# lbcb-sci/raven

Hardware: NVIDIA H100
Metric: overlaps/s (higher is better)
Workload: dtype u64

## Files before the change

raven_b200/csrc/capi.cu:

```cuda
#include <algorithm>
#include <cstring>

#include "engine.cuh"

using namespace rvn;

struct rvn_ctx {
  Ctx c;
};

namespace {

template <typename F>
int Guard(rvn_ctx* ctx, F&& f, bool sketches_first = false) {
  if (!ctx) return RVN_ERR_INVALID;
  try {
    RVN_CUDA(cudaSetDevice(ctx->c.device));
    if (!sketches_first) WaitUpload(ctx->c);
    f(ctx->c);
    ctx->c.err.clear();
    return RVN_OK;
  } catch (const InvalidArgument& e) {
    ctx->c.err = e.what();
    return RVN_ERR_INVALID;
// ... 677 lines not shown
    if (!out) throw InvalidArgument("null stats");
    *out = c.stats;
    out->occurrence = c.occurrence;
    out->kernel_launches = c.launches;
  }, true);
}

RVN_API int rvn_set_option(rvn_ctx* ctx, const char* name, int64_t value) {
  return Guard(ctx, [&](Ctx& c) {
    if (name && std::strcmp(name, "keep_hits") == 0) {
      c.keep_hits = value != 0;
    } else if (name && std::strcmp(name, "async_upload") == 0) {
      c.async_upload = value != 0;
    } else if (name && std::strcmp(name, "self_join") == 0) {
      c.self_join = value != 0;
    } else if (name && std::strcmp(name, "tier_min_records") == 0) {
      c.tier_min_records = value < 0 ? 0 : static_cast<uint64_t>(value);
    } else if (name && std::strcmp(name, "reset_stats") == 0) {
      std::memset(&c.stats, 0, sizeof(c.stats));
      c.launches = 0;
      TimerReset(c);
    } else {
      throw InvalidArgument("unknown option");
    }
  }, true);
}

RVN_API int rvn_get_timings(rvn_ctx* ctx, const char* const** names,
                            const float** ms, uint32_t* n) {
  return Guard(ctx, [&](Ctx& c) {
// ... 203 lines not shown
```

raven_b200/csrc/engine.cuh:

```cuda
#pragma once

#include <string>
#include <vector>

#include "../../include/raven_b200.h"
#include "common.cuh"

namespace rvn {

struct Params {
  uint32_t k = 15, w = 5, bandwidth = 500, chain = 4, matches = 100;
  uint32_t gap = 10000;
};

constexpr uint32_t kSketchTile = 2048;
constexpr uint32_t kSketchThreads = 256;
constexpr uint32_t kMaxWindow = 256;

struct PhaseTimer {
  std::vector<const char*> names;
  std::vector<float> ms;
  std::vector<std::pair<cudaEvent_t, cudaEvent_t>> pending;
  std::vector<cudaEvent_t> pool;
};
// ... 40 lines not shown

  bool q_valid = false;
  uint32_t q_first = 0, q_last = 0;
  uint64_t q_n = 0;
  DevBuf<uint64_t> q_val, q_org, q_off;
  bool q_is32 = false;
  std::vector<uint64_t> h_q_off;
  bool qt_valid = false;
  uint32_t qt_first = 0, qt_last = 0;
  DevBuf<uint64_t> qt_val;
  DevBuf<uint32_t> qt_pos;
  int t_b_low = 0;
  uint64_t group_count_min = 0;
  bool i_from_sketch = false;
  int64_t self_join = 1;

  bool i_valid = false;
  uint32_t i_first = 0, i_last = 0;
  uint64_t i_n = 0, i_keys = 0;
  DevBuf<uint64_t> i_val, i_org, i_val_alt, i_org_alt;
  bool i_is32 = false;
  int i_shift = 0;
  uint64_t i_limit = ~0ULL;
  DevBuf<uint32_t> t_cnt;
  DevBuf<uint64_t> t_off, t_aval, t_aorg, t_b0, t_b1, t_b2, t_narrow;
  const uint32_t* t_sorted_b = nullptr;
  uint64_t t_nb = 0;
  uint64_t tier_min_records = 1ULL << 18;
  DevBuf<uint32_t> i_bucket;
  int i_bucket_bits = 0;
  DevBuf<uint64_t> i_gaps;
  DevBuf<uint64_t> i_hist;
  uint32_t occurrence = 0xFFFFFFFFu;
  bool i_sorted_ids = false;
  bool ids_ascending = true;
  DevBuf<uint8_t> sort_tmp;

  DevBuf<uint32_t> m_cnt, m_first;
  DevBuf<uint8_t> m_filt;
  DevBuf<uint64_t> m_hit_off;
  DevBuf<uint64_t> m_sq_key, m_sq_key2;
  DevBuf<uint32_t> m_sq_idx, m_sq_idx2;
// ... 91 lines not shown
void TimerBegin(Ctx& c, const char* name);
void TimerEnd(Ctx& c);
void TimerCollect(Ctx& c);
void TimerReset(Ctx& c);

void EnsureTiles(Ctx& c);
void EnsureSketch(Ctx& c, uint32_t first, uint32_t last);
void WaitUpload(Ctx& c);
void EnsureMicromizers(Ctx& c, uint32_t first, uint32_t last);
void EnsureThresholds(Ctx& c, uint32_t first, uint32_t last);

void BuildIndex(Ctx& c, uint32_t first, uint32_t last, bool minhash,
                uint64_t value_limit = ~0ULL);
uint64_t MaxMicromizerValue(Ctx& c, uint32_t first, uint32_t last);
void BuildIndexFrom(Ctx& c, ValView src_val, const uint64_t* src_org, uint64_t n,
                    uint64_t index_bases, uint64_t value_limit = ~0ULL);

int RadixSortPairs(Ctx& c, const uint32_t* src_keys, uint32_t* keys_a, uint32_t* keys_b,
                   const uint64_t* src_vals, uint64_t* vals_a, uint64_t* vals_b, uint64_t n,
                   int begin_bit, int end_bit, bool descending = false);
int RadixSortPairs(Ctx& c, const uint64_t* src_keys, uint64_t* keys_a, uint64_t* keys_b,
                   const uint64_t* src_vals, uint64_t* vals_a, uint64_t* vals_b, uint64_t n,
                   int begin_bit, int end_bit, bool descending = false);
int RadixSortPairs(Ctx& c, const uint32_t* src_keys, uint32_t* keys_a, uint32_t* keys_b,
                   const uint32_t* src_vals, uint32_t* vals_a, uint32_t* vals_b, uint64_t n,
                   int begin_bit, int end_bit, bool descending = false);
int RadixSortPairs(Ctx& c, const uint64_t* src_keys, uint64_t* keys_a, uint64_t* keys_b,
                   const uint32_t* src_vals, uint32_t* vals_a, uint32_t* vals_b, uint64_t n,
                   int begin_bit, int end_bit, bool descending = false);
int RadixSortKeys(Ctx& c, const uint32_t* src_keys, uint32_t* keys_a, uint32_t* keys_b,
                  uint64_t n, int begin_bit, int end_bit);
uint64_t* IndexHistogram(Ctx& c);
uint32_t ThresholdFromHistogram(Ctx& c, const uint64_t* h_hist, uint64_t n_keys,
                                double frequency, bool* needs_long_runs);
uint32_t FilterIndex(Ctx& c, double frequency);

void MapRange(Ctx& c, uint32_t first, uint32_t last, bool avoid_equal,
              bool avoid_symmetric, bool minhash, bool want_filtered,
              bool fetch = true);

uint64_t ChainGroupedHits(Ctx& c, const uint64_t* hg, const uint64_t* hp,
                          const uint64_t* read_hit_off,
                          const std::vector<uint64_t>& h_rho, const uint32_t* lhs_ids,
                          uint32_t nr, uint64_t n_hits, uint64_t n_q);

void GatherReset(Ctx& c);
// ... 52 lines not shown
```

raven_b200/csrc/index.cu:

```cuda
#include <algorithm>
#include <cmath>

#include "engine.cuh"

namespace rvn {

namespace {

constexpr int kThreads = 256;

constexpr uint32_t kHistBins = 1u << 16;
constexpr uint32_t kSmemBins = 1024;

constexpr uint32_t kShortGap = 1024;
constexpr uint32_t kMaxLongGaps = 1u << 20;

template <typename ValT, bool kFill>
__global__ void __launch_bounds__(kThreads)
IndexTableKernel(const ValT* __restrict__ val, uint64_t n, int shift,
                 uint32_t n_buckets, uint32_t* __restrict__ bucket,
                 unsigned long long* __restrict__ hist, uint64_t* __restrict__ gaps) {
  __shared__ uint32_t sh[kSmemBins];
  __shared__ uint32_t keys;
  __shared__ uint32_t warp_first[kThreads / 32];
// ... 313 lines not shown
    atomicAdd(&sh[1], h1);
    atomicAdd(&sh[2], h2);
    atomicAdd(&sh[3], h3);
    atomicAdd(&sh[4], h4);
    atomicAdd(&keys_total, nkeys);
  }
  __syncthreads();
  for (uint32_t i = threadIdx.x; i < kSmemBins; i += kThreads) {
    if (sh[i]) atomicAdd(&hist[i], static_cast<unsigned long long>(sh[i]));
  }
  if (threadIdx.x == 0 && keys_total) {
    atomicAdd(&hist[kHistBins], static_cast<unsigned long long>(keys_total));
  }
}

}

uint64_t MaxMicromizerValue(Ctx& c, uint32_t first, uint32_t last) {
  EnsureThresholds(c, first, last);
  if (last <= first) return 0;
  if (!c.s_is32) return ~0ULL;
  uint64_t* w = c.m_counter.reserve(8);
  RVN_CUDA(cudaMemsetAsync(w, 0, sizeof(uint64_t), c.stream));
  const uint64_t n = last - first;
  MaxU64Kernel<<<std::min<unsigned>(CeilDiv(n, 256), c.sms * 8), 256, 0, c.stream>>>(
      c.qt_val.get(), n, reinterpret_cast<unsigned long long*>(w));
  RVN_LAUNCH_CHECK();
  ++c.launches;
  return ReadU64(c, w);
}
// ... 3 lines not shown
  c.occurrence = 0xFFFFFFFFu;
  EnsureSketch(c, first, last);
  ValView src_val{c.s_val.get(), c.s_is32 ? 1 : 0};
  const uint64_t* src_org = c.s_org.get();
  uint64_t n = c.s_n;
  if (minhash) {
    EnsureMicromizers(c, first, last);
    src_val = ValView{c.q_val.get(), c.q_is32 ? 1 : 0};
    src_org = c.q_org.get();
    n = c.q_n;
  }
  uint64_t bases = 0;
  for (uint32_t r = first; r < last; ++r) bases += c.h_len[r];
  c.i_first = first;
  c.i_last = last;
  BuildIndexFrom(c, src_val, src_org, n, bases, minhash ? ~0ULL : value_limit);
  c.i_sorted_ids = c.ids_ascending;
  c.i_from_sketch = !minhash;
}

void BuildIndexFrom(Ctx& c, ValView src_val, const uint64_t* src_org, uint64_t n,
                    uint64_t index_bases, uint64_t value_limit) {
  c.i_valid = false;
  c.i_sorted_ids = false;
  c.i_from_sketch = false;
  c.occurrence = 0xFFFFFFFFu;
  ++c.i_gen;
  if (n >= 0xFFFFFFFFULL) {
    throw LimitError("index batch holds 2^32 or more minimizers");
  }
  c.i_n = n;
  c.i_keys = 0;
  if (!src_val.is32 && 2 * c.prm.k <= 30 && n > 0) {
    uint32_t* narrow = reinterpret_cast<uint32_t*>(c.t_narrow.reserve(n / 2 + 2));
    NarrowValuesKernel<<<CeilDiv(n, kThreads), kThreads, 0, c.stream>>>(
        static_cast<const uint64_t*>(src_val.p), n, narrow);
    RVN_LAUNCH_CHECK();
    ++c.launches;
    src_val = ValView{narrow, 1};
  }
  const bool is32 = src_val.is32 != 0;
  c.i_is32 = is32;

  const int key_bits = static_cast<int>(2 * c.prm.k);
  const uint64_t value_mask = key_bits >= 64 ? ~0ULL : ((1ULL << key_bits) - 1);
  const bool tiered = is32 && value_limit < value_mask && n >= c.tier_min_records;
  const uint32_t limit32 = static_cast<uint32_t>(value_limit);
  c.i_limit = tiered ? value_limit : ~0ULL;
  uint64_t n_a = n, n_b = 0;
  const uint32_t* sorted_b = nullptr;

  TimerBegin(c, "index_sort");
  if (tiered) {
    const uint32_t* src32 = static_cast<const uint32_t*>(src_val.p);
    const uint64_t tiles = (n + kTierTile - 1) / kTierTile;
    uint32_t* tcnt = c.t_cnt.reserve(tiles + 1);
    uint64_t* toff = c.t_off.reserve(tiles + 2);
    TierCountKernel<<<static_cast<unsigned>(tiles), kThreads, 0, c.stream>>>(src32, n, limit32,
                                                                          tcnt);
    ExclusiveScanU32(c, tcnt, toff, tiles);
    n_a = ReadU64(c, toff + tiles);
    n_b = n - n_a;
    uint32_t* a_val = reinterpret_cast<uint32_t*>(c.t_aval.reserve(n_a / 2 + 2));
    uint64_t* a_org = c.t_aorg.reserve(n_a + 1);
    uint32_t* b_src = reinterpret_cast<uint32_t*>(c.t_b0.reserve(n_b / 2 + 2));
// ... 5 lines not shown
    while (bits_a < key_bits && (value_limit >> bits_a) != 0) ++bits_a;
    c.i_val.reserve(n_a / 2 + 2);
    c.i_val_alt.reserve(n_a / 2 + 2);
    c.i_org.reserve(n_a + 1);
    c.i_org_alt.reserve(n_a + 1);
    if (n_a > 0) {
      const int where = RadixSortPairs(c, a_val, reinterpret_cast<uint32_t*>(c.i_val.get()),
                                       reinterpret_cast<uint32_t*>(c.i_val_alt.get()), a_org,
                                       c.i_org.get(), c.i_org_alt.get(), n_a, 0, bits_a);
      if (where == 1) {
        c.i_val.swap(c.i_val_alt);
        c.i_org.swap(c.i_org_alt);
      }
    }
    uint32_t* b1 = reinterpret_cast<uint32_t*>(c.t_b1.reserve(n_b / 2 + 2));
    uint32_t* b2 = reinterpret_cast<uint32_t*>(c.t_b2.reserve(n_b / 2 + 2));
    const uint64_t n_groups = ((value_mask - value_limit) >> kGroupLowBits) + 1;
    c.t_b_low = (key_bits > 2 * kGroupLowBits && n_b / n_groups >= c.group_count_min)
                    ? kGroupLowBits
                    : 0;
    if (n_b > 0) {
      const int where = RadixSortKeys(c, b_src, b1, b2, n_b, c.t_b_low, key_bits);
      sorted_b = where < 0 ? b_src : (where == 0 ? b1 : b2);
    }
    c.t_sorted_b = sorted_b;
    c.t_nb = n_b;
  } else {
    const uint64_t val_elems = is32 ? n / 2 + 2 : n + 1;
    c.i_val.reserve(val_elems);
    c.i_val_alt.reserve(val_elems);
    c.i_org.reserve(n + 1);
    c.i_org_alt.reserve(n + 1);
    if (n > 0) {
      int where;
      if (is32) {
        where = RadixSortPairs(c, static_cast<const uint32_t*>(src_val.p),
                               reinterpret_cast<uint32_t*>(c.i_val.get()),
                               reinterpret_cast<uint32_t*>(c.i_val_alt.get()), src_org,
                               c.i_org.get(), c.i_org_alt.get(), n, 0, key_bits);
      } else {
        where = RadixSortPairs(c, static_cast<const uint64_t*>(src_val.p), c.i_val.get(),
                               c.i_val_alt.get(), src_org, c.i_org.get(), c.i_org_alt.get(), n, 0,
                               key_bits);
      }
      if (where == 1) {
        c.i_val.swap(c.i_val_alt);
        c.i_org.swap(c.i_org_alt);
      }
    }
    c.t_sorted_b = nullptr;
    c.t_nb = 0;
  }
  c.i_n = n_a;
  TimerEnd(c);
  const uint64_t* kv = c.i_val.get();

  TimerBegin(c, "index_table");
  int top_bits = key_bits;
  if (tiered) {
    top_bits = 1;
    while (top_bits < key_bits && (value_limit >> top_bits) != 0) ++top_bits;
  }
  int bits = 8;
  while (bits < 28 && (1ULL << (bits + 1)) <= n_a) ++bits;
  bits = std::min<int>(bits, top_bits);
  c.i_bucket_bits = bits;
  const int shift = top_bits - bits;
  c.i_shift = shift;
  const uint32_t n_buckets =
      tiered ? static_cast<uint32_t>((value_limit >> shift) + 1) : (1u << bits);
  uint32_t* bucket = c.i_bucket.reserve(n_buckets + 2ULL);
  static_assert(sizeof(unsigned long long) == sizeof(uint64_t), "");
  uint64_t* hist = c.i_hist.reserve(kHistBins + 8);
  RVN_CUDA(cudaMemsetAsync(hist, 0, (kHistBins + 8) * sizeof(uint64_t), c.stream));
  uint64_t* gaps = c.i_gaps.reserve(3ULL * kMaxLongGaps);
  const unsigned grid = std::min<unsigned>(CeilDiv(n_a + 1, kThreads), c.sms * 8);
  if (is32) {
    IndexTableKernel<uint32_t, true><<<grid, kThreads, 0, c.stream>>>(
        reinterpret_cast<const uint32_t*>(kv), n_a, shift, n_buckets, bucket,
        reinterpret_cast<unsigned long long*>(hist), gaps);
    if (tiered && n_b > 0) {
      if (c.t_b_low) {
        GroupCountKernel<<<std::min<unsigned>(CeilDiv(n_b, kGroupChunk * (kThreads / 32)), c.sms * 6),
                           kThreads, 0, c.stream>>>(sorted_b, n_b,
                                                    reinterpret_cast<unsigned long long*>(hist));
      } else {
        IndexTableKernel<uint32_t, false>
            <<<std::min<unsigned>(CeilDiv(n_b + 1, kThreads), c.sms * 8), kThreads, 0, c.stream>>>(
                sorted_b, n_b, 0, 0, nullptr, reinterpret_cast<unsigned long long*>(hist), nullptr);
      }
      ++c.launches;
    }
  } else {
    IndexTableKernel<uint64_t, true><<<grid, kThreads, 0, c.stream>>>(
        kv, n_a, shift, n_buckets, bucket, reinterpret_cast<unsigned long long*>(hist), gaps);
  }
  RVN_LAUNCH_CHECK();
// ... 54 lines not shown
  bool long_runs = false;
  uint32_t occ = ThresholdFromHistogram(c, h.data(), c.i_keys, frequency, &long_runs);
  if (long_runs) {
    uint64_t cum = 0;
    for (uint32_t len = 0; len + 1 < kHistBins; ++len) cum += h[len];
    std::size_t rank = static_cast<std::size_t>((1 - frequency) * static_cast<double>(c.i_keys));
    if (rank >= c.i_keys) rank = c.i_keys - 1;
    const uint64_t n_long = h[kHistBins - 1];
    uint32_t* out = c.m_cnt.reserve(n_long + 1);
    uint64_t* counter = c.m_counter.reserve(8);
    RVN_CUDA(cudaMemsetAsync(counter, 0, sizeof(uint64_t), c.stream));
    if (c.i_is32) {
      CollectLongRuns<uint32_t><<<CeilDiv(c.i_n, kThreads), kThreads, 0, c.stream>>>(
          reinterpret_cast<const uint32_t*>(c.i_val.get()), c.i_n,
          reinterpret_cast<unsigned long long*>(counter), out);
      if (c.t_sorted_b && c.t_nb && c.t_b_low) {
        uint32_t* bufs[3] = {reinterpret_cast<uint32_t*>(c.t_b0.get()),
                             reinterpret_cast<uint32_t*>(c.t_b1.get()),
                             reinterpret_cast<uint32_t*>(c.t_b2.get())};
        uint32_t* free_buf[2];
        int nf = 0;
        for (uint32_t* p : bufs) {
          if (p != c.t_sorted_b && nf < 2) free_buf[nf++] = p;
        }
        const int where = RadixSortKeys(c, c.t_sorted_b, free_buf[0], free_buf[1], c.t_nb, 0,
                                        static_cast<int>(2 * c.prm.k));
        c.t_sorted_b = where < 0 ? c.t_sorted_b : (where == 0 ? free_buf[0] : free_buf[1]);
        c.t_b_low = 0;
      }
      if (c.t_sorted_b && c.t_nb) {
        CollectLongRuns<uint32_t><<<CeilDiv(c.t_nb, kThreads), kThreads, 0, c.stream>>>(
            c.t_sorted_b, c.t_nb, reinterpret_cast<unsigned long long*>(counter), out);
      }
    } else {
      CollectLongRuns<uint64_t><<<CeilDiv(c.i_n, kThreads), kThreads, 0, c.stream>>>(
          c.i_val.get(), c.i_n, reinterpret_cast<unsigned long long*>(counter), out);
    }
    RVN_LAUNCH_CHECK();
    ++c.launches;
    std::vector<uint32_t> lens(n_long);
    RVN_CUDA(cudaMemcpyAsync(lens.data(), out, n_long * sizeof(uint32_t),
                             cudaMemcpyDeviceToHost, c.stream));
    RVN_CUDA(cudaStreamSynchronize(c.stream));
// ... 10 lines not shown
```

raven_b200/csrc/radix.cu:

```cuda
#include <algorithm>

#include "engine.cuh"

namespace rvn {

namespace {

constexpr int kRadixMaxBits = 10;
constexpr int kBins = 1 << kRadixMaxBits;
constexpr int kThreads = 256;
constexpr int kWarps = kThreads / 32;
constexpr int kBinsPerThread = kBins / kThreads;
constexpr int kMaxPasses = 8;
template <typename KeyT>
struct Items {
  static constexpr int value = sizeof(KeyT) == 4 ? 32 : 16;
};

constexpr uint32_t kFlagAggregate = 1u << 30;
constexpr uint32_t kFlagPrefix = 2u << 30;
constexpr uint32_t kFlagMask = 3u << 30;
constexpr uint32_t kValueMask = ~kFlagMask;

struct PassPlan {
// ... 31 lines not shown
  for (int i = threadIdx.x; i < total; i += kThreads) {
    if (sh_hist[i]) atomicAdd(&hist[i], static_cast<unsigned long long>(sh_hist[i]));
  }
}

__global__ void __launch_bounds__(kBins)
RadixScanBinsKernel(const unsigned long long* __restrict__ hist, int n_passes,
                    uint32_t* __restrict__ bin_base) {
  __shared__ uint32_t sm[34];
  for (int p = 0; p < n_passes; ++p) {
    const uint32_t v = static_cast<uint32_t>(hist[p * kBins + threadIdx.x]);
    uint32_t total;
    const uint32_t ex = BlockExclusiveSum<uint32_t, kBins>(v, sm, &total);
    bin_base[p * kBins + threadIdx.x] = ex;
  }
}

template <typename KeyT, typename ValT, bool HAS_VAL>
struct __align__(16) PassSmem {
  static constexpr int kTile = kThreads * Items<KeyT>::value;
  uint16_t warp_hist[kWarps][kBins];
  uint32_t bin_off[kBins];
  uint32_t bin_dst[kBins];
  uint32_t scan[34];
  uint32_t tile;
  uint16_t slot_digit[HAS_VAL ? kTile : 2];
  union {
    KeyT keys[kTile];
    ValT vals[HAS_VAL ? kTile : 1];
  } stage;
// ... 85 lines not shown
      sm.warp_hist[w][b] = static_cast<uint16_t>(c);
      c += x;
    }
    cnt[j] = c;
    mine += c;
  }
  uint32_t total;
  uint32_t ex = BlockExclusiveSum<uint32_t, kThreads>(mine, sm.scan, &total);
#pragma unroll
  for (int j = 0; j < kBinsPerThread; ++j) {
    sm.bin_off[threadIdx.x * kBinsPerThread + j] = ex;
    ex += cnt[j];
  }

  {
    uint4* st4 = reinterpret_cast<uint4*>(status);
    const uint64_t my4 = static_cast<uint64_t>(tile) * (kBins / 4) + threadIdx.x;
    uint32_t excl[kBinsPerThread] = {0, 0, 0, 0};
    static_assert(kBinsPerThread == 4, "one uint4 of status words per thread");
    if (tile > 0) {
      uint4 agg;
      agg.x = kFlagAggregate | cnt[0];
      agg.y = kFlagAggregate | cnt[1];
      agg.z = kFlagAggregate | cnt[2];
      agg.w = kFlagAggregate | cnt[3];
      asm volatile("st.volatile.global.v4.u32 [%0], {%1, %2, %3, %4};" ::"l"(st4 + my4),
                   "r"(agg.x), "r"(agg.y), "r"(agg.z), "r"(agg.w)
                   : "memory");
      constexpr int kLook = 4;
      uint32_t open = 0xF;
      int64_t p = static_cast<int64_t>(tile) - 1;
      while (open) {
        uint4 v[kLook];
#pragma unroll
        for (int u = 0; u < kLook; ++u) {
          const int64_t q = p - u;
          if (q >= 0) {
            const uint4* src = st4 + static_cast<uint64_t>(q) * (kBins / 4) + threadIdx.x;
            asm volatile("ld.volatile.global.v4.u32 {%0, %1, %2, %3}, [%4];"
                         : "=r"(v[u].x), "=r"(v[u].y), "=r"(v[u].z), "=r"(v[u].w)
                         : "l"(src)
                         : "memory");
          } else {
            v[u] = make_uint4(kFlagPrefix, kFlagPrefix, kFlagPrefix, kFlagPrefix);
          }
        }
        int used = 0;
#pragma unroll
        for (int u = 0; u < kLook; ++u) {
          const uint32_t vv[4] = {v[u].x, v[u].y, v[u].z, v[u].w};
          const bool ready = (vv[0] & kFlagMask) && (vv[1] & kFlagMask) && (vv[2] & kFlagMask) &&
                             (vv[3] & kFlagMask);
          if (used == u && ready && open) {
#pragma unroll
            for (int j = 0; j < kBinsPerThread; ++j) {
              if (open & (1u << j)) {
                excl[j] += vv[j] & kValueMask;
                if ((vv[j] & kFlagMask) == kFlagPrefix) open &= ~(1u << j);
              }
            }
            used = u + 1;
          }
        }
        p -= used;
      }
    }
    uint4 pre;
    pre.x = kFlagPrefix | (excl[0] + cnt[0]);
    pre.y = kFlagPrefix | (excl[1] + cnt[1]);
    pre.z = kFlagPrefix | (excl[2] + cnt[2]);
    pre.w = kFlagPrefix | (excl[3] + cnt[3]);
    asm volatile("st.volatile.global.v4.u32 [%0], {%1, %2, %3, %4};" ::"l"(st4 + my4), "r"(pre.x),
                 "r"(pre.y), "r"(pre.z), "r"(pre.w)
                 : "memory");
#pragma unroll
    for (int j = 0; j < kBinsPerThread; ++j) {
      const uint32_t b = threadIdx.x * kBinsPerThread + j;
      const uint32_t base = bin_base[b];
      sm.bin_dst[b] = base + excl[j] - sm.bin_off[b];
      if (tile == gridDim.x - 1) bin_next[b] = base + excl[j] + cnt[j];
    }
  }
  __syncthreads();

#pragma unroll
  for (int i = 0; i < kItems; ++i) {
    const uint32_t t = warp_base + i * 32 + lane;
    if (t < tile_count) {
      const uint32_t d = Digit<KeyT>(key[i], flip, begin_bit, dmask);
// ... 29 lines not shown
    __syncthreads();
  }

#pragma unroll
  for (int i = 0; i < kItems; ++i) {
    const uint32_t t = warp_base + i * 32 + lane;
    if (t < tile_count) sm.stage.keys[rank[i]] = key[i];
  }
  __syncthreads();
#pragma unroll
  for (int i = 0; i < kItems; ++i) {
    const uint32_t s = i * kThreads + threadIdx.x;
    if (s < tile_count) {
      const KeyT k = sm.stage.keys[s];
      keys_out[sm.bin_dst[Digit<KeyT>(k, flip, begin_bit, dmask)] + s] = k;
    }
  }
}

PassPlan MakePlan(int begin_bit, int end_bit) {
  PassPlan plan{};
  const int total = std::max(0, end_bit - begin_bit);
  const int np = (total + kRadixMaxBits - 1) / kRadixMaxBits;
  if (np > kMaxPasses) throw InvalidArgument("radix sort: too many key bits");
  plan.n_passes = np;
  int at = begin_bit;
  for (int p = 0; p < np; ++p) {
    const int b = (total - (at - begin_bit) + (np - p) - 1) / (np - p);
    plan.begin[p] = at;
    plan.bits[p] = b;
// ... 89 lines not shown
  return SortImpl<uint32_t, uint32_t, true>(c, src_keys, keys_a, keys_b, src_vals, vals_a, vals_b,
                                            n, begin_bit, end_bit, descending);
}
int RadixSortPairs(Ctx& c, const uint64_t* src_keys, uint64_t* keys_a, uint64_t* keys_b,
                   const uint32_t* src_vals, uint32_t* vals_a, uint32_t* vals_b, uint64_t n,
                   int begin_bit, int end_bit, bool descending) {
  return SortImpl<uint64_t, uint32_t, true>(c, src_keys, keys_a, keys_b, src_vals, vals_a, vals_b,
                                            n, begin_bit, end_bit, descending);
}
int RadixSortKeys(Ctx& c, const uint32_t* src_keys, uint32_t* keys_a, uint32_t* keys_b, uint64_t n,
                  int begin_bit, int end_bit) {
  return SortImpl<uint32_t, uint32_t, false>(c, src_keys, keys_a, keys_b, nullptr, nullptr, nullptr,
                                             n, begin_bit, end_bit, false);
}

}
```

Baseline: 52.78 million.

## Count tier-B index keys with a cluster shared-memory histogram instead of sorting

When building a tiered index, the bare tier-B keys are no longer fully radix-sorted. They get a single 10-bit radix partition into buckets, and a thread-block-cluster kernel then counts occurrences per key. It uses distributed shared memory reductions (mapa plus red.cluster) and feeds the occurrence histogram directly. This is meant to replace the multi-pass sort of tier B with one partition pass and a counting sweep. The tradeoff is that the B keys are left unsorted (t_b_sorted=false), which downstream paths must handle, and it adds cluster launch configuration and a new option.

```diff
diff --git a/profiles/index_build_split.py b/profiles/index_build_split.py
--- /dev/null
+++ b/profiles/index_build_split.py
@@ -0,0 +1,147 @@
+from __future__ import annotations
+
+import argparse
+import ctypes as C
+import json
+import os
+import subprocess
+import sys
+
+ROOT = os.path.dirname(os.path.dirname(os.path.abspath(__file__)))
+sys.path.insert(0, ROOT)
+
+SEED = 20260924
+K, W, FREQ, KMAX = 15, 5, 0.001, 32
+READS, GENOME, MEAN_LEN = 200_000, 50_000_000, 10_000
+
+KERNELS = ("TierCountKernel", "TierScatterKernel", "RadixHistogramKernel", "RadixScanBinsKernel",
+           "OnesweepPass", "PartitionPass", "GroupCountKernel", "BareCountKernel",
+           "IndexTableKernel", "FillLongGaps")
+
+
+def card():
+    try:
+        out = subprocess.run(["nvidia-smi", "--query-gpu=name,power.limit,clocks.max.sm",
+                              "--format=csv,noheader"], capture_output=True, text=True,
+                             timeout=30).stdout.strip().splitlines()
+        return out[0] if out else "unknown"
+    except (OSError, subprocess.SubprocessError):
+        return "unknown"
+
+
+def index_sizes(eng):
+    v, o, n, nk = (C.POINTER(C.c_uint64)(), C.POINTER(C.c_uint64)(), C.c_uint64(0),
+                   C.c_uint64(0))
+    eng._check(eng.lib.rvn_index_records(eng.h, C.byref(v), C.byref(o), C.byref(n), C.byref(nk)))
+    n_a = n.value
+    vmax = max(v[n_a - 1], 1) if n_a else 1
+    return n_a, int(eng.stats()["index_records"]), int(vmax).bit_length()
+
+
+def algorithmic_bytes(name, n, n_a, n_b, passes_a):
+    if "TierCountKernel" in name:
+        return 4 * n
+    if "TierScatterKernel" in name:
+        return 4 * n + 8 * n_a + 12 * n_a + 4 * n_b
+    if "RadixHistogramKernel<unsigned int>" in name:
+        return 4 * (n_a + n_b)
+    if "OnesweepPass<unsigned int, unsigned long" in name:
+        return passes_a * 24 * n_a
+    if "OnesweepPass<unsigned int, unsigned int, false>" in name:
+        return 2 * 8 * n_b
+    if "PartitionPass" in name:
+        return 8 * n_b
+    if "GroupCountKernel" in name or "BareCountKernel" in name:
+        return 4 * n_b
+    if "IndexTableKernel<unsigned int, true>" in name:
+        return 4 * n_a
+    return None
+
+
+def main():
+    ap = argparse.ArgumentParser()
+    ap.add_argument("--steps", type=int, default=3)
+    ap.add_argument("--warmup", type=int, default=2)
+    ap.add_argument("--bare-count", default="0,1,8,16")
+    ap.add_argument("--out", default=None, metavar="DIR",
+                    help="also write the tables as DIR/index_build_split.json")
+    a = ap.parse_args()
+
+    import torch
+    from torch.profiler import ProfilerActivity, profile
+
+    if not torch.cuda.is_available():
+        raise SystemExit("index_build_split.py needs a CUDA device")
+    from bench import synth
+    from raven_b200 import engine
+
+    rs = synth.make_reads(SEED, GENOME, READS, MEAN_LEN)
+    stream = torch.cuda.current_stream()
+    eng = engine.Engine(device=0, stream=stream.cuda_stream)
+    eng.configure(K, W)
+    eng.upload(rs)
+
+    def step():
+        eng.find_overlaps_and_create_piles(FREQ, KMAX, False, 0, fetch=False)
+
+    dev = card()
+    print(f"card: {dev}")
+    report = {"card": dev, "settings": {}}
+    for setting in a.bare_count.split(","):
+        if setting != "default":
+            eng.set_option("bare_count", int(setting))
+        for _ in range(a.warmup):
+            step()
+        torch.cuda.synchronize()
+        eng.set_option("reset_stats", 1)
+        with profile(activities=[ProfilerActivity.CUDA]) as prof:
+            for _ in range(a.steps):
+                step()
+            torch.cuda.synchronize()
+        phases = eng.timings()
+        free, total = torch.cuda.mem_get_info()
+        n_a, n, bits_a = index_sizes(eng)
+        n_b = n - n_a
+        passes_a = -(-bits_a // 10)
+        per = {}
+        for e in prof.events():
+            if e.device_type != torch.autograd.DeviceType.CUDA:
+                continue
+            if not any(k in e.name for k in KERNELS):
+                continue
+            d = per.setdefault(e.name, [0.0, 0])
+            d[0] += (e.time_range.end - e.time_range.start) / 1e3
+            d[1] += 1
+        rows = []
+        for name, (ms, cnt) in sorted(per.items(), key=lambda x: -x[1][0]):
+            ms_step, launches = ms / a.steps, cnt / a.steps
+            b = algorithmic_bytes(name, n, n_a, n_b, passes_a)
+            rate = (b / (ms_step * 1e-3) / 1e12) if b and ms_step > 0 else None
+            short = name.replace("(anonymous namespace)::", "").replace("void ", "")
+            short = short.replace("unsigned ", "u").replace("rvn::", "").split("(")[0]
+            rows.append({"kernel": short, "ms_per_step": round(ms_step, 3),
+                         "launches_per_step": launches,
+                         "gbytes": None if b is None else round(b / 1e9, 3),
+                         "tb_per_s": None if rate is None else round(rate, 3)})
+        print(f"\nbare_count={setting}: {a.steps} steps, n={n} n_a={n_a} n_b={n_b} "
+              f"(tier A: {bits_a} bits, {passes_a} passes); device memory in use after the "
+              f"steps {(total - free) / 2**30:.2f} GiB")
+        print(f"  phases (last step, ms): index_sort {phases.get('index_sort', 0):.2f}  "
+              f"index_table {phases.get('index_table', 0):.2f}")
+        print(f"  {'kernel':<58} {'ms/step':>8} {'launch':>6} {'GB':>7} {'TB/s':>6}")
+        for r in rows:
+            print(f"  {r['kernel'][:58]:<58} {r['ms_per_step']:8.3f} {r['launches_per_step']:6.1f} "
+                  f"{'' if r['gbytes'] is None else r['gbytes']:>7} "
+                  f"{'' if r['tb_per_s'] is None else r['tb_per_s']:>6}")
+        report["settings"][setting] = {
+            "n": n, "n_a": n_a, "n_b": n_b, "phases_ms": phases, "kernels": rows,
+            "device_mem_used_gib": round((total - free) / 2**30, 3)}
+    if a.out:
+        os.makedirs(a.out, exist_ok=True)
+        with open(os.path.join(a.out, "index_build_split.json"), "w") as f:
+            json.dump(report, f, indent=1)
+    eng.close()
+
+
+if __name__ == "__main__":
+    main()
diff --git a/raven_b200/csrc/capi.cu b/raven_b200/csrc/capi.cu
--- a/raven_b200/csrc/capi.cu
+++ b/raven_b200/csrc/capi.cu
@@ -715,6 +715,12 @@
       c.async_upload = value != 0;
     } else if (name && std::strcmp(name, "self_join") == 0) {
       c.self_join = value != 0;
+    } else if (name && std::strcmp(name, "bare_count") == 0) {
+      if (value != 0 && value != 1 && value != 8 && value != 16) {
+        throw InvalidArgument("bare_count: 0, 1, 8 or 16");
+      }
+      c.bare_count = value;
+      c.bare_cluster = 0;
     } else if (name && std::strcmp(name, "tier_min_records") == 0) {
       c.tier_min_records = value < 0 ? 0 : static_cast<uint64_t>(value);
     } else if (name && std::strcmp(name, "reset_stats") == 0) {
diff --git a/raven_b200/csrc/engine.cuh b/raven_b200/csrc/engine.cuh
--- a/raven_b200/csrc/engine.cuh
+++ b/raven_b200/csrc/engine.cuh
@@ -78,6 +78,7 @@
   uint64_t group_count_min = 0;
   bool i_from_sketch = false;
   int64_t self_join = 1;
+  int64_t bare_count = 1;
 
   bool i_valid = false;
   uint32_t i_first = 0, i_last = 0;
@@ -90,6 +91,10 @@
   DevBuf<uint64_t> t_off, t_aval, t_aorg, t_b0, t_b1, t_b2, t_narrow;
   const uint32_t* t_sorted_b = nullptr;
   uint64_t t_nb = 0;
+  bool t_b_sorted = true;
+  DevBuf<uint32_t> t_bstart;
+  int bare_cluster = 0;
+  int bare_clusters = 0;
   uint64_t tier_min_records = 1ULL << 18;
   DevBuf<uint32_t> i_bucket;
   int i_bucket_bits = 0;
@@ -211,7 +216,7 @@
                 uint64_t value_limit = ~0ULL);
 uint64_t MaxMicromizerValue(Ctx& c, uint32_t first, uint32_t last);
 void BuildIndexFrom(Ctx& c, ValView src_val, const uint64_t* src_org, uint64_t n,
-                    uint64_t index_bases, uint64_t value_limit = ~0ULL);
+                    uint64_t index_bases, uint64_t value_limit = ~0ULL, bool count_bare = false);
 
 int RadixSortPairs(Ctx& c, const uint32_t* src_keys, uint32_t* keys_a, uint32_t* keys_b,
                    const uint64_t* src_vals, uint64_t* vals_a, uint64_t* vals_b, uint64_t n,
@@ -227,6 +232,8 @@
                    int begin_bit, int end_bit, bool descending = false);
 int RadixSortKeys(Ctx& c, const uint32_t* src_keys, uint32_t* keys_a, uint32_t* keys_b,
                   uint64_t n, int begin_bit, int end_bit);
+void RadixPartitionKeys(Ctx& c, const uint32_t* src, uint32_t* dst, uint64_t n, int begin_bit,
+                        int end_bit, uint32_t* bin_start);
 uint64_t* IndexHistogram(Ctx& c);
 uint32_t ThresholdFromHistogram(Ctx& c, const uint64_t* h_hist, uint64_t n_keys,
                                 double frequency, bool* needs_long_runs);
diff --git a/raven_b200/csrc/index.cu b/raven_b200/csrc/index.cu
--- a/raven_b200/csrc/index.cu
+++ b/raven_b200/csrc/index.cu
@@ -1,5 +1,7 @@
 #include <algorithm>
 #include <cmath>
+
+#include <cooperative_groups.h>
 
 #include "engine.cuh"
 
@@ -351,6 +353,155 @@
   }
 }
 
+constexpr int kBareBucketBits = 10;
+constexpr int kBareThreads = 1024;
+constexpr int kBareSlotBits = 15;
+
+__global__ void __launch_bounds__(kBareThreads, 1)
+BareCountKernel(const uint32_t* __restrict__ key, uint64_t n, const uint32_t* __restrict__ bstart,
+                uint32_t first_bucket, uint32_t n_buckets, int span_bits, int slot_bits,
+                unsigned long long* __restrict__ hist) {
+  extern __shared__ __align__(16) uint32_t bare_smem[];
+  __shared__ uint32_t keys_total;
+  namespace cg = cooperative_groups;
+  cg::cluster_group cluster = cg::this_cluster();
+  const uint32_t csize = cluster.num_blocks();
+  const uint32_t crank = cluster.block_rank();
+  const uint32_t n_slots = 1u << slot_bits;
+  uint32_t* ctr = bare_smem;
+  uint32_t* sh = bare_smem + n_slots;
+  for (uint32_t i = threadIdx.x; i < n_slots; i += kBareThreads) ctr[i] = 0;
+  for (uint32_t i = threadIdx.x; i < kSmemBins; i += kBareThreads) sh[i] = 0;
+  if (threadIdx.x == 0) keys_total = 0;
+  const uint32_t ctr_addr = static_cast<uint32_t>(__cvta_generic_to_shared(ctr));
+  const uint32_t span_mask = (1u << span_bits) - 1u;
+  const uint32_t sweep_span = n_slots * csize;
+  const uint32_t slot_mask = n_slots - 1u;
+  uint32_t h1 = 0, h2 = 0, h3 = 0, h4 = 0, nkeys = 0;
+  cluster.sync();
+  const uint32_t n_clusters = gridDim.x / csize;
+  for (uint32_t b = first_bucket + blockIdx.x / csize; b < n_buckets; b += n_clusters) {
+    const uint64_t lo = bstart ? bstart[b] : 0;
+    const uint64_t hi = bstart && b + 1 < n_buckets ? bstart[b + 1] : n;
+    if (lo >= hi) continue;
+    for (uint64_t s0 = 0; s0 <= span_mask; s0 += sweep_span) {
+      constexpr int kUnroll = 4;
+      const uint64_t stride = static_cast<uint64_t>(csize) * kBareThreads;
+      for (uint64_t i0 = lo + crank * kBareThreads + threadIdx.x; i0 < hi; i0 += kUnroll * stride) {
+        uint32_t k4[kUnroll];
+#pragma unroll
+        for (int u = 0; u < kUnroll; ++u) {
+          const uint64_t i = i0 + u * stride;
+          k4[u] = i < hi ? key[i] : 0u;
+        }
+#pragma unroll
+        for (int u = 0; u < kUnroll; ++u) {
+          const uint64_t v = static_cast<uint64_t>(k4[u] & span_mask) - s0;
+          if (i0 + u * stride < hi && v < sweep_span) {
+            const uint32_t owner = static_cast<uint32_t>(v) >> slot_bits;
+            const uint32_t local = ctr_addr + 4u * (static_cast<uint32_t>(v) & slot_mask);
+            uint32_t remote;
+            asm volatile("mapa.shared::cluster.u32 %0, %1, %2;" : "=r"(remote) : "r"(local), "r"(owner));
+            asm volatile("red.relaxed.cluster.shared::cluster.add.u32 [%0], 1;" ::"r"(remote) : "memory");
+          }
+        }
+      }
+      cluster.sync();
+      for (uint32_t t = threadIdx.x; t < n_slots; t += kBareThreads) {
+        const uint32_t c = ctr[t];
+        if (c == 0) continue;
+        ctr[t] = 0;
+        ++nkeys;
+        if (c <= 4) {
+          h1 += c == 1;
+          h2 += c == 2;
+          h3 += c == 3;
+          h4 += c == 4;
+        } else if (c < kSmemBins) {
+          atomicAdd(&sh[c], 1u);
+        } else {
+          atomicAdd(&hist[min(c, kHistBins - 1)], 1ULL);
+        }
+      }
+      cluster.sync();
+    }
+  }
+#pragma unroll
+  for (int d = 16; d > 0; d >>= 1) {
+    h1 += __shfl_xor_sync(0xFFFFFFFFu, h1, d);
+    h2 += __shfl_xor_sync(0xFFFFFFFFu, h2, d);
+    h3 += __shfl_xor_sync(0xFFFFFFFFu, h3, d);
+    h4 += __shfl_xor_sync(0xFFFFFFFFu, h4, d);
+    nkeys += __shfl_xor_sync(0xFFFFFFFFu, nkeys, d);
+  }
+  if ((threadIdx.x & 31) == 0) {
+    atomicAdd(&sh[1], h1);
+    atomicAdd(&sh[2], h2);
+    atomicAdd(&sh[3], h3);
+    atomicAdd(&sh[4], h4);
+    atomicAdd(&keys_total, nkeys);
+  }
+  __syncthreads();
+  for (uint32_t i = threadIdx.x; i < kSmemBins; i += kBareThreads) {
+    if (sh[i]) atomicAdd(&hist[i], static_cast<unsigned long long>(sh[i]));
+  }
+  if (threadIdx.x == 0 && keys_total) {
+    atomicAdd(&hist[kHistBins], static_cast<unsigned long long>(keys_total));
+  }
+}
+
+void BareCount(Ctx& c, const uint32_t* keys, uint64_t n, int key_bits, uint32_t limit,
+               const uint32_t* bstart, unsigned long long* hist) {
+  const int span_bits = bstart ? key_bits - kBareBucketBits : key_bits;
+  const uint32_t n_buckets = bstart ? (1u << kBareBucketBits) : 1u;
+  const uint32_t first_bucket = bstart ? (limit >> span_bits) : 0u;
+  if (c.bare_cluster == 0) {
+    const int size = c.bare_count > 1 ? static_cast<int>(c.bare_count) : 8;
+    const size_t smem = ((1u << kBareSlotBits) + kSmemBins) * sizeof(uint32_t);
+    RVN_CUDA(cudaFuncSetAttribute(BareCountKernel, cudaFuncAttributeMaxDynamicSharedMemorySize,
+                                  static_cast<int>(smem)));
+    RVN_CUDA(cudaFuncSetAttribute(BareCountKernel, cudaFuncAttributeNonPortableClusterSizeAllowed, 1));
+    cudaLaunchConfig_t cfg = {};
+    cfg.gridDim = dim3(static_cast<unsigned>(size));
+    cfg.blockDim = dim3(kBareThreads);
+    cfg.dynamicSmemBytes = smem;
+    cudaLaunchAttribute attr[1];
+    attr[0].id = cudaLaunchAttributeClusterDimension;
+    attr[0].val.clusterDim.x = static_cast<unsigned>(size);
+    attr[0].val.clusterDim.y = 1;
+    attr[0].val.clusterDim.z = 1;
+    cfg.attrs = attr;
+    cfg.numAttrs = 1;
+    int clusters = 0;
+    RVN_CUDA(cudaOccupancyMaxActiveClusters(&clusters, BareCountKernel, &cfg));
+    if (clusters < 1) throw CudaError("BareCountKernel: a cluster does not fit the device");
+    c.bare_cluster = size;
+    c.bare_clusters = clusters;
+  }
+  const int csize = c.bare_cluster;
+  int log_c = 0;
+  while ((1 << log_c) < csize) ++log_c;
+  const int slot_bits = std::max(0, std::min(kBareSlotBits, span_bits - log_c));
+  const unsigned clusters =
+      static_cast<unsigned>(std::min<uint64_t>(n_buckets - first_bucket, c.bare_clusters));
+  cudaLaunchConfig_t cfg = {};
+  cfg.gridDim = dim3(clusters * csize);
+  cfg.blockDim = dim3(kBareThreads);
+  cfg.dynamicSmemBytes = ((1u << slot_bits) + kSmemBins) * sizeof(uint32_t);
+  cfg.stream = c.stream;
+  cudaLaunchAttribute attr[1];
+  attr[0].id = cudaLaunchAttributeClusterDimension;
+  attr[0].val.clusterDim.x = static_cast<unsigned>(csize);
+  attr[0].val.clusterDim.y = 1;
+  attr[0].val.clusterDim.z = 1;
+  cfg.attrs = attr;
+  cfg.numAttrs = 1;
+  RVN_CUDA(cudaLaunchKernelEx(&cfg, BareCountKernel, keys, n, bstart, first_bucket, n_buckets,
+                              span_bits, slot_bits, hist));
+  RVN_LAUNCH_CHECK();
+  ++c.launches;
+}
+
 }
 
 uint64_t MaxMicromizerValue(Ctx& c, uint32_t first, uint32_t last) {
@@ -384,13 +535,14 @@
   for (uint32_t r = first; r < last; ++r) bases += c.h_len[r];
   c.i_first = first;
   c.i_last = last;
-  BuildIndexFrom(c, src_val, src_org, n, bases, minhash ? ~0ULL : value_limit);
+  BuildIndexFrom(c, src_val, src_org, n, bases, minhash ? ~0ULL : value_limit,
+                 true);
   c.i_sorted_ids = c.ids_ascending;
   c.i_from_sketch = !minhash;
 }
 
 void BuildIndexFrom(Ctx& c, ValView src_val, const uint64_t* src_org, uint64_t n,
-                    uint64_t index_bases, uint64_t value_limit) {
+                    uint64_t index_bases, uint64_t value_limit, bool count_bare) {
   c.i_valid = false;
   c.i_sorted_ids = false;
   c.i_from_sketch = false;
@@ -419,6 +571,8 @@
   c.i_limit = tiered ? value_limit : ~0ULL;
   uint64_t n_a = n, n_b = 0;
   const uint32_t* sorted_b = nullptr;
+  const bool bare = tiered && count_bare && c.bare_count != 0;
+  const uint32_t* bstart = nullptr;
 
   TimerBegin(c, "index_sort");
   if (tiered) {
@@ -454,14 +608,28 @@
       }
     }
     uint32_t* b1 = reinterpret_cast<uint32_t*>(c.t_b1.reserve(n_b / 2 + 2));
-    uint32_t* b2 = reinterpret_cast<uint32_t*>(c.t_b2.reserve(n_b / 2 + 2));
-    const uint64_t n_groups = ((value_mask - value_limit) >> kGroupLowBits) + 1;
-    c.t_b_low = (key_bits > 2 * kGroupLowBits && n_b / n_groups >= c.group_count_min)
-                    ? kGroupLowBits
-                    : 0;
-    if (n_b > 0) {
-      const int where = RadixSortKeys(c, b_src, b1, b2, n_b, c.t_b_low, key_bits);
-      sorted_b = where < 0 ? b_src : (where == 0 ? b1 : b2);
+    if (bare) {
+      c.t_b2.release();
+      c.t_b_low = 0;
+      c.t_b_sorted = false;
+      sorted_b = n_b > 0 ? b_src : nullptr;
+      if (n_b > 0 && key_bits > 2 * kBareBucketBits) {
+        uint32_t* starts = c.t_bstart.reserve(1u << kBareBucketBits);
+        RadixPartitionKeys(c, b_src, b1, n_b, key_bits - kBareBucketBits, key_bits, starts);
+        sorted_b = b1;
+        bstart = starts;
+      }
+    } else {
+      uint32_t* b2 = reinterpret_cast<uint32_t*>(c.t_b2.reserve(n_b / 2 + 2));
+      const uint64_t n_groups = ((value_mask - value_limit) >> kGroupLowBits) + 1;
+      c.t_b_low = (key_bits > 2 * kGroupLowBits && n_b / n_groups >= c.group_count_min)
+                      ? kGroupLowBits
+                      : 0;
+      c.t_b_sorted = c.t_b_low == 0;
+      if (n_b > 0) {
+        const int where = RadixSortKeys(c, b_src, b1, b2, n_b, c.t_b_low, key_bits);
+        sorted_b = where < 0 ? b_src : (where == 0 ? b1 : b2);
+      }
     }
     c.t_sorted_b = sorted_b;
     c.t_nb = n_b;
@@ -490,6 +658,7 @@
     }
     c.t_sorted_b = nullptr;
     c.t_nb = 0;
+    c.t_b_sorted = true;
   }
   c.i_n = n_a;
   TimerEnd(c);
@@ -520,7 +689,11 @@
         reinterpret_cast<const uint32_t*>(kv), n_a, shift, n_buckets, bucket,
         reinterpret_cast<unsigned long long*>(hist), gaps);
     if (tiered && n_b > 0) {
-      if (c.t_b_low) {
+      if (bare) {
+        BareCount(c, sorted_b, n_b, key_bits, limit32, bstart,
+                  reinterpret_cast<unsigned long long*>(hist));
+        --c.launches;
+      } else if (c.t_b_low) {
         GroupCountKernel<<<std::min<unsigned>(CeilDiv(n_b, kGroupChunk * (kThreads / 32)), c.sms * 6),
                            kThreads, 0, c.stream>>>(sorted_b, n_b,
                                                     reinterpret_cast<unsigned long long*>(hist));
@@ -605,19 +778,20 @@
       CollectLongRuns<uint32_t><<<CeilDiv(c.i_n, kThreads), kThreads, 0, c.stream>>>(
           reinterpret_cast<const uint32_t*>(c.i_val.get()), c.i_n,
           reinterpret_cast<unsigned long long*>(counter), out);
-      if (c.t_sorted_b && c.t_nb && c.t_b_low) {
+      if (c.t_sorted_b && c.t_nb && !c.t_b_sorted) {
         uint32_t* bufs[3] = {reinterpret_cast<uint32_t*>(c.t_b0.get()),
                              reinterpret_cast<uint32_t*>(c.t_b1.get()),
                              reinterpret_cast<uint32_t*>(c.t_b2.get())};
-        uint32_t* free_buf[2];
-        int nf = 0;
+        uint32_t* src = nullptr;
         for (uint32_t* p : bufs) {
-          if (p != c.t_sorted_b && nf < 2) free_buf[nf++] = p;
-        }
-        const int where = RadixSortKeys(c, c.t_sorted_b, free_buf[0], free_buf[1], c.t_nb, 0,
+          if (p == c.t_sorted_b) src = p;
+        }
+        uint32_t* other = src == bufs[0] ? bufs[1] : bufs[0];
+        const int where = RadixSortKeys(c, src, other, src, c.t_nb, 0,
                                         static_cast<int>(2 * c.prm.k));
-        c.t_sorted_b = where < 0 ? c.t_sorted_b : (where == 0 ? free_buf[0] : free_buf[1]);
+        c.t_sorted_b = where == 0 ? other : src;
         c.t_b_low = 0;
+        c.t_b_sorted = true;
       }
       if (c.t_sorted_b && c.t_nb) {
         CollectLongRuns<uint32_t><<<CeilDiv(c.t_nb, kThreads), kThreads, 0, c.stream>>>(
diff --git a/raven_b200/csrc/radix.cu b/raven_b200/csrc/radix.cu
--- a/raven_b200/csrc/radix.cu
+++ b/raven_b200/csrc/radix.cu
@@ -69,6 +69,71 @@
     const uint32_t ex = BlockExclusiveSum<uint32_t, kBins>(v, sm, &total);
     bin_base[p * kBins + threadIdx.x] = ex;
   }
+}
+
+__device__ __forceinline__ void ChainTileCounts(uint32_t* __restrict__ status, uint32_t tile,
+                                                const uint32_t (&cnt)[kBinsPerThread],
+                                                uint32_t (&excl)[kBinsPerThread]) {
+  uint4* st4 = reinterpret_cast<uint4*>(status);
+  const uint64_t my4 = static_cast<uint64_t>(tile) * (kBins / 4) + threadIdx.x;
+#pragma unroll
+  for (int j = 0; j < kBinsPerThread; ++j) excl[j] = 0;
+  static_assert(kBinsPerThread == 4, "one uint4 of status words per thread");
+  if (tile > 0) {
+    uint4 agg;
+    agg.x = kFlagAggregate | cnt[0];
+    agg.y = kFlagAggregate | cnt[1];
+    agg.z = kFlagAggregate | cnt[2];
+    agg.w = kFlagAggregate | cnt[3];
+    asm volatile("st.volatile.global.v4.u32 [%0], {%1, %2, %3, %4};" ::"l"(st4 + my4),
+                 "r"(agg.x), "r"(agg.y), "r"(agg.z), "r"(agg.w)
+                 : "memory");
+    constexpr int kLook = 4;
+    uint32_t open = 0xF;
+    int64_t p = static_cast<int64_t>(tile) - 1;
+    while (open) {
+      uint4 v[kLook];
+#pragma unroll
+      for (int u = 0; u < kLook; ++u) {
+        const int64_t q = p - u;
+        if (q >= 0) {
+          const uint4* src = st4 + static_cast<uint64_t>(q) * (kBins / 4) + threadIdx.x;
+          asm volatile("ld.volatile.global.v4.u32 {%0, %1, %2, %3}, [%4];"
+                       : "=r"(v[u].x), "=r"(v[u].y), "=r"(v[u].z), "=r"(v[u].w)
+                       : "l"(src)
+                       : "memory");
+        } else {
+          v[u] = make_uint4(kFlagPrefix, kFlagPrefix, kFlagPrefix, kFlagPrefix);
+        }
+      }
+      int used = 0;
+#pragma unroll
+      for (int u = 0; u < kLook; ++u) {
+        const uint32_t vv[4] = {v[u].x, v[u].y, v[u].z, v[u].w};
+        const bool ready = (vv[0] & kFlagMask) && (vv[1] & kFlagMask) && (vv[2] & kFlagMask) &&
+                           (vv[3] & kFlagMask);
+        if (used == u && ready && open) {
+#pragma unroll
+          for (int j = 0; j < kBinsPerThread; ++j) {
+            if (open & (1u << j)) {
+              excl[j] += vv[j] & kValueMask;
+              if ((vv[j] & kFlagMask) == kFlagPrefix) open &= ~(1u << j);
+            }
+          }
+          used = u + 1;
+        }
+      }
+      p -= used;
+    }
+  }
+  uint4 pre;
+  pre.x = kFlagPrefix | (excl[0] + cnt[0]);
+  pre.y = kFlagPrefix | (excl[1] + cnt[1]);
+  pre.z = kFlagPrefix | (excl[2] + cnt[2]);
+  pre.w = kFlagPrefix | (excl[3] + cnt[3]);
+  asm volatile("st.volatile.global.v4.u32 [%0], {%1, %2, %3, %4};" ::"l"(st4 + my4), "r"(pre.x),
+               "r"(pre.y), "r"(pre.z), "r"(pre.w)
+               : "memory");
 }
 
 template <typename KeyT, typename ValT, bool HAS_VAL>
@@ -184,65 +249,8 @@
   }
 
   {
-    uint4* st4 = reinterpret_cast<uint4*>(status);
-    const uint64_t my4 = static_cast<uint64_t>(tile) * (kBins / 4) + threadIdx.x;
-    uint32_t excl[kBinsPerThread] = {0, 0, 0, 0};
-    static_assert(kBinsPerThread == 4, "one uint4 of status words per thread");
-    if (tile > 0) {
-      uint4 agg;
-      agg.x = kFlagAggregate | cnt[0];
-      agg.y = kFlagAggregate | cnt[1];
-      agg.z = kFlagAggregate | cnt[2];
-      agg.w = kFlagAggregate | cnt[3];
-      asm volatile("st.volatile.global.v4.u32 [%0], {%1, %2, %3, %4};" ::"l"(st4 + my4),
-                   "r"(agg.x), "r"(agg.y), "r"(agg.z), "r"(agg.w)
-                   : "memory");
-      constexpr int kLook = 4;
-      uint32_t open = 0xF;
-      int64_t p = static_cast<int64_t>(tile) - 1;
-      while (open) {
-        uint4 v[kLook];
-#pragma unroll
-        for (int u = 0; u < kLook; ++u) {
-          const int64_t q = p - u;
-          if (q >= 0) {
-            const uint4* src = st4 + static_cast<uint64_t>(q) * (kBins / 4) + threadIdx.x;
-            asm volatile("ld.volatile.global.v4.u32 {%0, %1, %2, %3}, [%4];"
-                         : "=r"(v[u].x), "=r"(v[u].y), "=r"(v[u].z), "=r"(v[u].w)
-                         : "l"(src)
-                         : "memory");
-          } else {
-            v[u] = make_uint4(kFlagPrefix, kFlagPrefix, kFlagPrefix, kFlagPrefix);
-          }
-        }
-        int used = 0;
-#pragma unroll
-        for (int u = 0; u < kLook; ++u) {
-          const uint32_t vv[4] = {v[u].x, v[u].y, v[u].z, v[u].w};
-          const bool ready = (vv[0] & kFlagMask) && (vv[1] & kFlagMask) && (vv[2] & kFlagMask) &&
-                             (vv[3] & kFlagMask);
-          if (used == u && ready && open) {
-#pragma unroll
-            for (int j = 0; j < kBinsPerThread; ++j) {
-              if (open & (1u << j)) {
-                excl[j] += vv[j] & kValueMask;
-                if ((vv[j] & kFlagMask) == kFlagPrefix) open &= ~(1u << j);
-              }
-            }
-            used = u + 1;
-          }
-        }
-        p -= used;
-      }
-    }
-    uint4 pre;
-    pre.x = kFlagPrefix | (excl[0] + cnt[0]);
-    pre.y = kFlagPrefix | (excl[1] + cnt[1]);
-    pre.z = kFlagPrefix | (excl[2] + cnt[2]);
-    pre.w = kFlagPrefix | (excl[3] + cnt[3]);
-    asm volatile("st.volatile.global.v4.u32 [%0], {%1, %2, %3, %4};" ::"l"(st4 + my4), "r"(pre.x),
-                 "r"(pre.y), "r"(pre.z), "r"(pre.w)
-                 : "memory");
+    uint32_t excl[kBinsPerThread];
+    ChainTileCounts(status, tile, cnt, excl);
 #pragma unroll
     for (int j = 0; j < kBinsPerThread; ++j) {
       const uint32_t b = threadIdx.x * kBinsPerThread + j;
@@ -302,6 +310,97 @@
     if (s < tile_count) {
       const KeyT k = sm.stage.keys[s];
       keys_out[sm.bin_dst[Digit<KeyT>(k, flip, begin_bit, dmask)] + s] = k;
+    }
+  }
+}
+
+struct PartitionSmem {
+  uint32_t bin_cnt[kBins];
+  uint32_t bin_off[kBins];
+  uint32_t bin_dst[kBins];
+  uint32_t scan[34];
+  uint32_t tile;
+  uint32_t keys[kThreads * Items<uint32_t>::value];
+};
+
+__global__ void __launch_bounds__(kThreads, 2)
+PartitionPass(const uint32_t* __restrict__ keys_in, uint32_t* __restrict__ keys_out, uint32_t n,
+              int begin_bit, int pass_bits, const uint32_t* __restrict__ bin_base,
+              uint32_t* __restrict__ bin_next, uint32_t* __restrict__ status,
+              unsigned int* __restrict__ ticket) {
+  extern __shared__ __align__(16) unsigned char smem_raw[];
+  PartitionSmem& sm = *reinterpret_cast<PartitionSmem*>(smem_raw);
+  constexpr int kItems = Items<uint32_t>::value;
+  constexpr int kTile = kThreads * kItems;
+  constexpr int kWarpTile = 32 * kItems;
+  const uint32_t lane = threadIdx.x & 31, warp = threadIdx.x >> 5;
+  const uint32_t dmask = (1u << pass_bits) - 1u;
+
+  if (threadIdx.x == 0) sm.tile = atomicAdd(ticket, 1u);
+#pragma unroll
+  for (int j = 0; j < kBinsPerThread; ++j) sm.bin_cnt[j * kThreads + threadIdx.x] = 0;
+  __syncthreads();
+  const uint32_t tile = sm.tile;
+  const uint64_t tile_base = static_cast<uint64_t>(tile) * kTile;
+  const uint32_t tile_count =
+      static_cast<uint32_t>(min(static_cast<uint64_t>(kTile), static_cast<uint64_t>(n) - tile_base));
+
+  uint32_t key[kItems];
+  const uint32_t warp_base = warp * kWarpTile;
+#pragma unroll
+  for (int i = 0; i < kItems; ++i) {
+    const uint32_t t = warp_base + i * 32 + lane;
+    key[i] = t < tile_count ? keys_in[tile_base + t] : 0u;
+  }
+  uint16_t rank[kItems];
+#pragma unroll
+  for (int i = 0; i < kItems; ++i) {
+    const uint32_t t = warp_base + i * 32 + lane;
+    if (t < tile_count) {
+      rank[i] = static_cast<uint16_t>(atomicAdd(&sm.bin_cnt[(key[i] >> begin_bit) & dmask], 1u));
+    }
+  }
+  __syncthreads();
+
+  uint32_t cnt[kBinsPerThread];
+  uint32_t mine = 0;
+#pragma unroll
+  for (int j = 0; j < kBinsPerThread; ++j) {
+    cnt[j] = sm.bin_cnt[threadIdx.x * kBinsPerThread + j];
+    mine += cnt[j];
+  }
+  uint32_t total;
+  uint32_t ex = BlockExclusiveSum<uint32_t, kThreads>(mine, sm.scan, &total);
+#pragma unroll
+  for (int j = 0; j < kBinsPerThread; ++j) {
+    sm.bin_off[threadIdx.x * kBinsPerThread + j] = ex;
+    ex += cnt[j];
+  }
+  {
+    uint32_t excl[kBinsPerThread];
+    ChainTileCounts(status, tile, cnt, excl);
+#pragma unroll
+    for (int j = 0; j < kBinsPerThread; ++j) {
+      const uint32_t b = threadIdx.x * kBinsPerThread + j;
+      const uint32_t base = bin_base[b];
+      sm.bin_dst[b] = base + excl[j] - sm.bin_off[b];
+      if (tile == gridDim.x - 1) bin_next[b] = base + excl[j] + cnt[j];
+    }
+  }
+  __syncthreads();
+
+#pragma unroll
+  for (int i = 0; i < kItems; ++i) {
+    const uint32_t t = warp_base + i * 32 + lane;
+    if (t < tile_count) sm.keys[sm.bin_off[(key[i] >> begin_bit) & dmask] + rank[i]] = key[i];
+  }
+  __syncthreads();
+#pragma unroll
+  for (int i = 0; i < kItems; ++i) {
+    const uint32_t s = i * kThreads + threadIdx.x;
+    if (s < tile_count) {
+      const uint32_t k = sm.keys[s];
+      keys_out[sm.bin_dst[(k >> begin_bit) & dmask] + s] = k;
     }
   }
 }
@@ -421,4 +520,60 @@
                                              n, begin_bit, end_bit, false);
 }
 
-}
+void RadixPartitionKeys(Ctx& c, const uint32_t* src, uint32_t* dst, uint64_t n, int begin_bit,
+                        int end_bit, uint32_t* bin_start) {
+  if (n >= 0xFFFFFFFFULL) throw LimitError("radix partition of 2^32 or more records");
+  if (end_bit - begin_bit < 1 || end_bit - begin_bit > kRadixMaxBits) {
+    throw InvalidArgument("radix partition: 1 to 10 key bits");
+  }
+  PassPlan plan{};
+  plan.n_passes = 1;
+  plan.begin[0] = begin_bit;
+  plan.bits[0] = end_bit - begin_bit;
+  constexpr uint64_t kTile = kThreads * Items<uint32_t>::value;
+  const uint64_t portion = ((1ULL << 30) - 1) / kTile * kTile;
+  const uint64_t n_portions = (n + portion - 1) / portion;
+  const uint64_t max_tiles = (std::min(n, portion) + kTile - 1) / kTile;
+  const size_t hist_bytes = sizeof(uint64_t) * kBins;
+  const size_t base_bytes = sizeof(uint32_t) * kBins;
+  const size_t ticket_bytes = sizeof(unsigned int) * kMaxPasses * 8;
+  if (n_portions > kMaxPasses * 8) throw LimitError("radix partition: too many launches");
+  const size_t head = hist_bytes + 2 * base_bytes + ticket_bytes;
+  const size_t status_bytes = sizeof(uint32_t) * max_tiles * kBins;
+  uint8_t* scratch = c.sort_tmp.reserve(head + status_bytes + 256);
+  auto* hist = reinterpret_cast<unsigned long long*>(scratch);
+  uint32_t* bases[2] = {reinterpret_cast<uint32_t*>(scratch + hist_bytes),
+                        reinterpret_cast<uint32_t*>(scratch + hist_bytes + base_bytes)};
+  auto* ticket = reinterpret_cast<unsigned int*>(scratch + hist_bytes + 2 * base_bytes);
+  auto* status = reinterpret_cast<uint32_t*>(scratch + head);
+  RVN_CUDA(cudaMemsetAsync(scratch, 0, head, c.stream));
+  if (n == 0) {
+    RVN_CUDA(cudaMemsetAsync(bin_start, 0, base_bytes, c.stream));
+    return;
+  }
+  const unsigned hgrid =
+      static_cast<unsigned>(std::min<uint64_t>((n + kThreads - 1) / kThreads, c.sms * 8));
+  RadixHistogramKernel<uint32_t><<<hgrid, kThreads, sizeof(uint32_t) * kBins, c.stream>>>(
+      src, n, plan, 0u, hist);
+  RadixScanBinsKernel<<<1, kBins, 0, c.stream>>>(hist, 1, bases[0]);
+  RVN_LAUNCH_CHECK();
+  c.launches += 2;
+  RVN_CUDA(cudaMemcpyAsync(bin_start, bases[0], base_bytes, cudaMemcpyDeviceToDevice, c.stream));
+  RVN_CUDA(cudaFuncSetAttribute(PartitionPass, cudaFuncAttributeMaxDynamicSharedMemorySize,
+                                static_cast<int>(sizeof(PartitionSmem))));
+  int cur = 0;
+  for (uint64_t q = 0; q < n_portions; ++q) {
+    const uint64_t first = q * portion;
+    const uint64_t cnt = std::min(portion, n - first);
+    const uint64_t tiles = (cnt + kTile - 1) / kTile;
+    RVN_CUDA(cudaMemsetAsync(status, 0, sizeof(uint32_t) * tiles * kBins, c.stream));
+    PartitionPass<<<static_cast<unsigned>(tiles), kThreads, sizeof(PartitionSmem), c.stream>>>(
+        src + first, dst, static_cast<uint32_t>(cnt), plan.begin[0], plan.bits[0], bases[cur],
+        bases[cur ^ 1], status, ticket + q);
+    RVN_LAUNCH_CHECK();
+    ++c.launches;
+    cur ^= 1;
+  }
+}
+
+}
```

Result: faster. 55.62 million (median of 6 runs) (+5.4%).
